# florianwechsung/alfi

Measured on AMD Instinct MI355X. Metric: V-cycles/sec on ldc3d P2-P0 (DoF*smooths/sec in dof_smooths_per_s), higher is better.
Workload: dtype f64

## Files before the change

### alfi_amd/_lib.py

```python
import ctypes
import os

from . import env

_HERE = os.path.dirname(os.path.abspath(__file__))
LIB_PATH = env.hip_lib() or os.path.join(_HERE, "libalfi_hip.so")

c_i32p = ctypes.POINTER(ctypes.c_int32)
c_i64p = ctypes.POINTER(ctypes.c_int64)
c_f64p = ctypes.POINTER(ctypes.c_double)
vp = ctypes.c_void_p


class CsrHost(ctypes.Structure):
    _fields_ = [("nrows", ctypes.c_int64), ("ncols", ctypes.c_int64), ("rowptr", vp), ("colidx", vp), ("vals", vp)]


class BsrHost(ctypes.Structure):
    _fields_ = [("nbrows", ctypes.c_int64), ("nbcols", ctypes.c_int64), ("rowptr", vp), ("colidx", vp), ("vals", vp)]


SIGNATURES = {
    "alfi_ctx_create": (ctypes.c_int, [ctypes.c_int, vp, ctypes.POINTER(vp)]),
    "alfi_ctx_destroy": (ctypes.c_int, [vp]),
# ... 57 lines not shown
    "alfi_level_set_facet_beta": (ctypes.c_int, [vp, vp, ctypes.c_double]),
    "alfi_level_assemble_burman": (ctypes.c_int, [vp, ctypes.c_double, ctypes.c_double, ctypes.c_double, vp, ctypes.c_double,
                                                  ctypes.c_int]),
    "alfi_level_transpose": (ctypes.c_int, [vp]),
    "alfi_level_get_values": (ctypes.c_int, [vp, vp]),
    "alfi_level_size": (ctypes.c_int, [vp, ctypes.POINTER(ctypes.c_int64)]),
    "alfi_spmv": (ctypes.c_int, [vp, vp, vp]),
    "alfi_residual": (ctypes.c_int, [vp, vp, vp, vp]),
    "alfi_patches_set": (ctypes.c_int, [vp, ctypes.c_int64, vp, vp]),
    "alfi_patches_factor": (ctypes.c_int, [vp]),
    "alfi_patches_set_groups": (ctypes.c_int, [vp, vp]),
    "alfi_patches_factor_bytes": (ctypes.c_int, [vp, ctypes.POINTER(ctypes.c_int64)]),
    "alfi_patches_find_groups": (ctypes.c_int, [vp, vp]),
    "alfi_ctx_set_condense_min_bytes": (ctypes.c_int, [vp, ctypes.c_int64]),
    "alfi_patches_condensed": (ctypes.c_int, [vp, ctypes.POINTER(ctypes.c_int)]),
    "alfi_patches_set_storage": (ctypes.c_int, [vp, ctypes.c_int]),
    "alfi_patches_storage": (ctypes.c_int, [vp, ctypes.POINTER(ctypes.c_int)]),
    "alfi_patches_set_macro_storage": (ctypes.c_int, [vp, ctypes.c_int]),
    "alfi_ctx_set_f32_work_bytes": (ctypes.c_int, [vp, ctypes.c_int64]),
    "alfi_ctx_f32_work_bytes": (ctypes.c_int, [vp, ctypes.POINTER(ctypes.c_int64)]),
    "alfi_patches_set_canonical_order": (ctypes.c_int, [vp, vp]),
    "alfi_patch_apply_split": (ctypes.c_int, [vp, ctypes.c_int64, vp, vp]),
    "alfi_patches_check": (ctypes.c_int, [vp, ctypes.POINTER(ctypes.c_double), ctypes.POINTER(ctypes.c_int64),
                                          ctypes.POINTER(ctypes.c_int64), ctypes.POINTER(ctypes.c_double)]),
    "alfi_patches_set_partition_of_unity": (ctypes.c_int, [vp, ctypes.c_int]),
    "alfi_patches_set_multiplicative": (ctypes.c_int, [vp, ctypes.c_int64, vp, ctypes.c_int]),
    "alfi_patches_multiplicative_levels": (ctypes.c_int, [vp, ctypes.POINTER(ctypes.c_int64)]),
    "alfi_patch_apply": (ctypes.c_int, [vp, vp, vp]),
    "alfi_patches_stats": (ctypes.c_int, [vp, ctypes.POINTER(ctypes.c_int64), ctypes.POINTER(ctypes.c_int64),
                                          ctypes.POINTER(ctypes.c_int64)]),
# ... 110 lines not shown
```

### alfi_amd/csrc/api_patches.hip

```cpp
#include <optional>
#include "api_internal.h"
#include "find_groups.h"

static_assert(PLAN_E_ARG == ALFI_E_ARG, "the planners (patch_plan.h) return the C ABI's code");


static void free_f32(alfi_level* L) {
  if (L->inv32 && --L->ctx->f32_levels == 0) {
    dev_free(L->ctx->f32_work);
    L->ctx->f32_work = nullptr;
    L->ctx->f32_work_doubles = 0;
  }
  dev_free(L->inv32);
  dev_free(L->inv32_ptr);
  L->inv32 = nullptr;
  L->inv32_ptr = nullptr;
  L->inv32_floats = 0;
  std::vector<int64_t>().swap(L->f32_ptr);
  if (L->held == HELD_F32) set_held(L, HELD_NONE);
}

static int inv_to_placeholder(alfi_level* L) {
  dev_free(L->inv);
  L->inv = nullptr;
// ... 216 lines not shown
  return 0;
}

int alfi_patches_find_groups(alfi_level* L, int32_t* group_out) {
  alfi_ctx* ctx = L->ctx;
  if (!L->patch_ptr) return alfi_set_error(ctx, ALFI_E_STATE, "alfi_patches_find_groups before alfi_patches_set");
  if (!group_out) return alfi_set_error(ctx, ALFI_E_ARG, "group_out is NULL");
  return find_groups(L, group_out, nullptr);
}

int alfi_ctx_set_condense_min_bytes(alfi_ctx* ctx, int64_t min_bytes) {
  ctx->condense_min_bytes = min_bytes;
  return 0;
}

int alfi_patches_condensed(alfi_level* L, int* mode) {
  if (mode) *mode = !L->cond ? 0 : (cond_by_own_choice(L) ? 2 : 1);
  return 0;
}

int alfi_patches_factor_bytes(alfi_level* L, int64_t* bytes) {
  if (L->held == HELD_F32) {
    *bytes = 4 * L->inv32_floats;
  } else if (wants_f32(L)) {
    std::vector<int64_t> ptr;
    *bytes = 4 * plan_f32_offsets(L->npatch, L->lay.patch_ptr.data(), &ptr);
  } else {
    *bytes = L->cond ? 8 * (L->cplan.mat_doubles + L->cplan.sinv_doubles) : 8 * L->lay.inv_doubles;
  }
  return 0;
// ... 336 lines not shown
```

### alfi_amd/csrc/common.h

```cpp
#pragma once
#include <hip/hip_runtime.h>
#include <atomic>
#include <cstdint>
#include <cstdio>
#include <string>
#include <thread>
#include <vector>
#include "alfi_hip.h"
#include "env.h"
#include "patch_plan.h"

inline std::atomic<int64_t> g_alfi_h2d_bytes{0}, g_alfi_d2h_bytes{0};
inline hipError_t alfi_counted_memcpy(void* dst, const void* src, size_t n, hipMemcpyKind kind) {
  if (kind == hipMemcpyHostToDevice) g_alfi_h2d_bytes += (int64_t)n;
  else if (kind == hipMemcpyDeviceToHost) g_alfi_d2h_bytes += (int64_t)n;
  return hipMemcpy(dst, src, n, kind);
}
inline hipError_t alfi_counted_memcpy_async(void* dst, const void* src, size_t n, hipMemcpyKind kind, hipStream_t s) {
  if (kind == hipMemcpyHostToDevice) g_alfi_h2d_bytes += (int64_t)n;
  else if (kind == hipMemcpyDeviceToHost) g_alfi_d2h_bytes += (int64_t)n;
  return hipMemcpyAsync(dst, src, n, kind, s);
}
#define hipMemcpy(dst, src, n, kind) alfi_counted_memcpy(dst, src, n, kind)
#define hipMemcpyAsync(dst, src, n, kind, stream) alfi_counted_memcpy_async(dst, src, n, kind, stream)
// ... 14 lines not shown
    const int64_t a = t * step, b = a + step < n ? a + step : n;
    if (a < b) th.emplace_back([&fn, a, b] { fn(a, b); });
  }
  fn((int64_t)0, step < n ? step : n);
  for (auto& t : th) t.join();
}

struct alfi_ctx {
  int device = 0;
  hipStream_t stream = nullptr;
  int64_t comm_nhalo = 0, comm_nred = 0, comm_sent = 0;
  int32_t* dev_err = nullptr;
  bool use_graph = false;
  bool block_kernels = true;
  bool block_fused = true;
  int block_lds_bytes = 64 * 1024;
  void* big_arena = nullptr;
  size_t big_arena_bytes = 0;
  void* asm_scratch = nullptr;
  size_t asm_scratch_bytes = 0;
  double* f32_work = nullptr;
  int64_t f32_work_doubles = 0;
  int f32_levels = 0;
  int64_t f32_work_cap = (int64_t)1 << 30;
  int64_t asm_scratch_limit = (int64_t)24 << 30;
  int64_t condense_min_bytes = alfi_default_condense_min_bytes();
  bool own_stream = false;
  std::string err;
  int prof = 0;
  struct EvPair {
// ... 541 lines not shown
```

### alfi_amd/csrc/cond_layout.h

```cpp
#pragma once
#include <cstdint>

#ifdef __HIPCC__
#define ALFI_HD __host__ __device__
#else
#define ALFI_HD
#endif

struct CondChunk {
  int64_t off;
  int64_t ubase;
  int64_t sidx0;
  int64_t stage_off;
  int32_t xq0, xq1;
  int32_t bq0, bq1;
  int32_t e0, ne;
  int32_t u0, nu;
  int32_t nI;
  int32_t xp0, bp0;
  int32_t pad;
};

#ifndef ALFI_COND_SIGMA_ROWS
#define ALFI_COND_SIGMA_ROWS 64
#endif
constexpr int COND_SIGMA_ROWS = ALFI_COND_SIGMA_ROWS;

constexpr int64_t COND_PER_PATCH_MIN = 1024;

ALFI_HD inline int cond_patch_waves(int max_pairs) {
#ifdef ALFI_COND_WAVES_FORCE
  (void)max_pairs;
  return ALFI_COND_WAVES_FORCE;
#else
  return max_pairs <= 64 ? 1 : max_pairs <= 128 ? 2 : max_pairs <= 256 ? 4 : 8;
#endif
}

ALFI_HD inline int cond_ldim(int rows) { return (rows + 1) & ~1; }
ALFI_HD inline int cond_pairs(int rows) { return (rows + 1) / 2; }
ALFI_HD inline int64_t cond_group_doubles(int m, int sc) {
  return (int64_t)cond_ldim(m) * m + (int64_t)cond_ldim(sc) * m + (int64_t)cond_ldim(m) * sc;
}
```

### alfi_amd/csrc/host_assemble.cpp

```cpp
#include <algorithm>
#include <cmath>
#include <cstdint>
#include <cstring>
#include <utility>
#include <vector>
#include <omp.h>

#include "find_groups.h"
#include "patch_plan.h"

extern "C" {

int alfi_host_node_graph(int64_t ncell, int nloc, const int32_t* cell_nodes, int64_t nnode, int32_t* rowptr,
                         int32_t* colidx) {
  std::vector<int64_t> nptr(nnode + 1, 0);
  for (int64_t c = 0; c < ncell; ++c)
    for (int a = 0; a < nloc; ++a) nptr[cell_nodes[c * nloc + a] + 1]++;
  for (int64_t i = 0; i < nnode; ++i) nptr[i + 1] += nptr[i];
  std::vector<int32_t> ncells(nptr[nnode]);
  {
    std::vector<int64_t> fill(nptr.begin(), nptr.end() - 1);
    for (int64_t c = 0; c < ncell; ++c)
      for (int a = 0; a < nloc; ++a) ncells[fill[cell_nodes[c * nloc + a]]++] = (int32_t)c;
  }
// ... 744 lines not shown
  ALFI_PLAN_TABLE(cond, dofs); ALFI_PLAN_TABLE(cond, slot); ALFI_PLAN_TABLE(cond, gptr); ALFI_PLAN_TABLE(cond, g_off);
  ALFI_PLAN_TABLE(cond, g_m); ALFI_PLAN_TABLE(cond, g_sc); ALFI_PLAN_TABLE(cond, g_uoff); ALFI_PLAN_TABLE(cond, g_mat);
  ALFI_PLAN_TABLE(cond, g_sidx); ALFI_PLAN_TABLE(cond, sidx); ALFI_PLAN_TABLE(cond, p_nI); ALFI_PLAN_TABLE(cond, sptr);
  ALFI_PLAN_TABLE(cond, sinv_ptr); ALFI_PLAN_TABLE(cond, s_uptr); ALFI_PLAN_TABLE(cond, s_uidx); ALFI_PLAN_TABLE(cond, order);
  ALFI_PLAN_TABLE(cond, chptr); ALFI_PLAN_TABLE(cond, ch_patch); ALFI_PLAN_TABLE(cond, ch_row); ALFI_PLAN_TABLE(cond, uptr);
  ALFI_PLAN_TABLE(cond, u_dst); ALFI_PLAN_TABLE(cond, xp_ptr); ALFI_PLAN_TABLE(cond, xp_grp); ALFI_PLAN_TABLE(cond, g_xp);
  ALFI_PLAN_TABLE(cond, bp_ptr); ALFI_PLAN_TABLE(cond, bp_grp); ALFI_PLAN_TABLE(cond, g_bp); ALFI_PLAN_TABLE(cond, gcptr);
  ALFI_PLAN_TABLE(cond, gc);
  ALFI_PLAN_SCALAR(cond, ngroups); ALFI_PLAN_SCALAR(cond, mat_doubles); ALFI_PLAN_SCALAR(cond, sinv_doubles);
  ALFI_PLAN_SCALAR(cond, lds_bytes); ALFI_PLAN_SCALAR(cond, lds_front);
  ALFI_PLAN_SCALAR(cond, lds_back); ALFI_PLAN_SCALAR(cond, lds_gfront); ALFI_PLAN_SCALAR(cond, lds_gback);
  ALFI_PLAN_SCALAR(cond, max_s); ALFI_PLAN_SCALAR(cond, max_m); ALFI_PLAN_SCALAR(cond, max_pairs); ALFI_PLAN_SCALAR(cond, umax);
  return h;
}

alfi_host_plan* alfi_host_plan_sweep(int bs, int64_t nbrows, int64_t npatch, const int64_t* patch_ptr, const int32_t* patch_dofs,
                                     const int32_t* rowptr, const int32_t* colidx, int64_t nit, const int64_t* iterset,
                                     int symmetrise) {
  alfi_host_plan* h = new alfi_host_plan();
  bool big = false;
  h->rc = check_sweep(bs, npatch, patch_ptr, patch_dofs, SMALL_PATCH_MAX, nit, iterset, &big, &h->err);
  if (h->rc == 0)
    h->rc = plan_sweep(bs, nbrows, npatch, patch_ptr, patch_dofs, rowptr, colidx, nit, iterset, symmetrise != 0, big, &h->sweep,
                       &h->err);
  if (h->rc != 0) return h;
  ALFI_PLAN_TABLE(sweep, seq); ALFI_PLAN_TABLE(sweep, wave_ptr); ALFI_PLAN_TABLE(sweep, items); ALFI_PLAN_TABLE(sweep, pred0);
  ALFI_PLAN_TABLE(sweep, succ_ptr); ALFI_PLAN_TABLE(sweep, succ); ALFI_PLAN_TABLE(sweep, rowtab);
  ALFI_PLAN_SCALAR(sweep, big); ALFI_PLAN_SCALAR(sweep, nitems);
  return h;
}
// ... 19 lines not shown
```

### alfi_amd/csrc/kernels_bigpatch.hip

```cpp
#include <algorithm>
#include <cstdlib>
#include <vector>
#include "common.h"
#include "row_piece.h"
#include "cond_apply.h"

constexpr int BIG_NB = 64;
constexpr int BIG_MAX_NP = PATCH_MAX;

template <int BS>
__global__ __launch_bounds__(256) void big_gather_kernel(int64_t p0, const int32_t* __restrict__ rowptr,
                                                          const int32_t* __restrict__ colidx,
                                                          const double* __restrict__ vals, int flat,
                                                          const int64_t* __restrict__ patch_ptr,
                                                          const int32_t* __restrict__ patch_dofs,
                                                          const int64_t* __restrict__ scr_ptr, double* __restrict__ scr) {
  __shared__ int32_t dofs_s[BIG_MAX_NP];
  const int64_t p = p0 + blockIdx.y;
  const int64_t off = patch_ptr[p];
  const int n = (int)(patch_ptr[p + 1] - off);
  const int N = (n + BIG_NB - 1) / BIG_NB * BIG_NB;
  double* S = scr + scr_ptr[blockIdx.y];
  for (int i = threadIdx.x; i < n; i += 256) dofs_s[i] = patch_dofs[off + i];
  const int chunk = (N + gridDim.x - 1) / gridDim.x;
// ... 751 lines not shown
    const double* B = cd.mat + cd.g_mat[g] + (int64_t)ldm * m;
    const double* W = B + (int64_t)ldsc * m;
    const int32_t* si = cd.sidx + cd.g_sidx[g];
    for (int e = threadIdx.x; e < sc * sc; e += 256) {
      const int i = e % sc, j = e / sc;
      double acc = 0.0;
      for (int k = 0; k < m; ++k) acc = __builtin_fma(B[(int64_t)k * ldsc + i], W[(int64_t)j * ldm + k], acc);
      S[(int64_t)si[i] * N + si[j]] -= acc;
    }
    __syncthreads();
  }
}



template <bool NT, int COND_WAVES, int RU>
__global__ __launch_bounds__(64 * COND_WAVES) void cond_front_kernel(int64_t p0, int64_t p1, CondDev cd,
                                                                     const int64_t* __restrict__ patch_ptr,
                                                                     const int64_t* __restrict__ stage_ptr,
                                                                     const double* __restrict__ x, double* __restrict__ stage,
                                                                     int ordered) {
  extern __shared__ double cond_dsmem[];
  constexpr int NT_ = 64 * COND_WAVES;
  if (p0 + blockIdx.x >= p1) return;
  const int64_t p = ordered ? cd.order[blockIdx.x] : p0 + blockIdx.x;
  const int64_t off = patch_ptr[p];
  const int n = (int)(patch_ptr[p + 1] - off);
  const int nI = cd.p_nI[p];
  const int s = n - nI;
  const int64_t uo0 = cd.uptr[p];
  double* xs = cond_dsmem;
  double* ts = xs + n;
  double* us = ts + nI;
  for (int i0 = threadIdx.x; i0 < n; i0 += 4 * NT_) {
    int32_t d[4];
#pragma unroll
    for (int u = 0; u < 4; ++u) d[u] = (i0 + u * NT_ < n) ? cd.dofs[off + i0 + u * NT_] : 0;
    double v[4];
#pragma unroll
    for (int u = 0; u < 4; ++u) v[u] = (i0 + u * NT_ < n) ? x[d[u]] : 0.0;
#pragma unroll
    for (int u = 0; u < 4; ++u)
      if (i0 + u * NT_ < n) xs[i0 + u * NT_] = v[u];
  }
  __syncthreads();
  double* tmp = cd.tmp + off;
  const int64_t xp0 = cd.xp_ptr[p], bp0 = cd.bp_ptr[p];
  const int nxp = (int)(cd.xp_ptr[p + 1] - xp0), nbp = (int)(cd.bp_ptr[p + 1] - bp0);
  for (int q0 = 0; q0 < nxp; q0 += NT_) {
    const int q = q0 + threadIdx.x;
    const bool act = q < nxp;
    const int32_t g = act ? cd.xp_grp[xp0 + q] : (int32_t)cd.gptr[p];
    const int m = cd.g_m[g], o = cd.g_off[g], i = 2 * (q - cd.g_xp[g]);
    double t0 = 0.0, t1 = 0.0;
    cond_row2_dot<NT, RU>(cd.mat + cd.g_mat[g] + i, cond_ldim(m), act ? m : 0, xs + o, t0, t1);
    if (act) {
      ts[o + i] = t0;
      tmp[o + i] = t0;
      if (i + 1 < m) {
        ts[o + i + 1] = t1;
        tmp[o + i + 1] = t1;
      }
    }
  }
  __syncthreads();
  for (int q0 = 0; q0 < nbp; q0 += NT_) {
    const int q = q0 + threadIdx.x;
    const bool act = q < nbp;
    const int32_t g = act ? cd.bp_grp[bp0 + q] : (int32_t)cd.gptr[p];
    const int m = cd.g_m[g], sc = cd.g_sc[g], j = 2 * (q - cd.g_bp[g]);
    const int64_t ue = uo0 + cd.g_uoff[g] + j;
    const int32_t d0 = act ? cd.u_dst[ue] : 0, d1 = (act && j + 1 < sc) ? cd.u_dst[ue + 1] : 0;
    double u0 = 0.0, u1 = 0.0;
    cond_row2_dot<NT, RU>(cd.mat + cd.g_mat[g] + (int64_t)cond_ldim(m) * m + j, cond_ldim(sc), act ? m : 0,
                          ts + cd.g_off[g], u0, u1);
    if (act) {
      us[d0] = u0;
      if (j + 1 < sc) us[d1] = u1;
    }
  }
  __syncthreads();
  const int64_t srow0 = cd.sptr[p];
  const int32_t qb = cd.s_uptr[srow0];
  double* rhs = stage + stage_ptr[p] + nI;
  for (int i = threadIdx.x; i < s; i += NT_) {
    double acc = xs[nI + i];
    const int32_t qe = cd.s_uptr[srow0 + i + 1] - qb;
    for (int32_t q = cd.s_uptr[srow0 + i] - qb; q < qe; ++q) acc -= us[q];
    rhs[i] = acc;
  }
}

template <bool NT>
__global__ __launch_bounds__(256) void cond_sigma_kernel(int64_t c0, CondDev cd, const int64_t* __restrict__ patch_ptr,
                                                         const int64_t* __restrict__ stage_ptr,
                                                         const double* __restrict__ stage) {
  extern __shared__ double cond_dsmem[];
  const int64_t c = c0 + blockIdx.x;
  const int64_t p = cd.ch_patch[c];
  const int r0 = cd.ch_row[c];
  const int64_t off = patch_ptr[p];
  const int n = (int)(patch_ptr[p + 1] - off);
  const int nI = cd.p_nI[p];
// ... 27 lines not shown
                                                                    const int64_t* __restrict__ stage_ptr,
                                                                    double* __restrict__ stage, int ordered) {
  extern __shared__ double cond_dsmem[];
  constexpr int NT_ = 64 * COND_WAVES;
  if (p0 + blockIdx.x >= p1) return;
  const int64_t p = ordered ? cd.order[blockIdx.x] : p0 + blockIdx.x;
  const int64_t off = patch_ptr[p];
  const int n = (int)(patch_ptr[p + 1] - off);
  const int nI = cd.p_nI[p];
  const int s = n - nI;
  const int uo = (int)(cd.uptr[p + 1] - cd.uptr[p]);
  const int64_t g0 = cd.gptr[p];
  double* ys = cond_dsmem;
  double* yg = ys + s;
  const double* tmp = cd.tmp + off;
  for (int i = threadIdx.x; i < s; i += NT_) ys[i] = tmp[nI + i];
  const int32_t* si = cd.sidx + (uo > 0 ? cd.g_sidx[g0] : 0);
  int32_t sq[4];
#pragma unroll
  for (int u = 0; u < 4; ++u) sq[u] = (threadIdx.x + u * NT_ < uo) ? si[threadIdx.x + u * NT_] : 0;
  __syncthreads();
#pragma unroll
  for (int u = 0; u < 4; ++u)
    if (threadIdx.x + u * NT_ < uo) yg[threadIdx.x + u * NT_] = ys[sq[u]];
  for (int q = threadIdx.x + 4 * NT_; q < uo; q += NT_) yg[q] = ys[si[q]];
  __syncthreads();
  double* out = stage + stage_ptr[p];
  const int64_t xp0 = cd.xp_ptr[p];
  const int nxp = (int)(cd.xp_ptr[p + 1] - xp0);
  for (int q0 = 0; q0 < nxp; q0 += NT_) {
    const int q = q0 + threadIdx.x;
    const bool act = q < nxp;
    const int32_t g = act ? cd.xp_grp[xp0 + q] : (int32_t)g0;
    const int m = cd.g_m[g], sc = cd.g_sc[g], o = cd.g_off[g], i = 2 * (q - cd.g_xp[g]);
    const int ldm = cond_ldim(m);
    const double tg0 = act ? tmp[o + i] : 0.0, tg1 = (act && i + 1 < m) ? tmp[o + i + 1] : 0.0;
    const int32_t sl0 = act ? cd.slot[off + o + i] : 0, sl1 = (act && i + 1 < m) ? cd.slot[off + o + i + 1] : 0;
    double y0 = 0.0, y1 = 0.0;
    cond_row2_dot<NT, RU>(cd.mat + cd.g_mat[g] + (int64_t)ldm * m + (int64_t)cond_ldim(sc) * m + i, ldm, act ? sc : 0,
                          yg + cd.g_uoff[g], y0, y1);
    if (act) {
      out[sl0] = tg0 - y0;
      if (i + 1 < m) out[sl1] = tg1 - y1;
    }
  }
  for (int i = threadIdx.x; i < s; i += NT_) out[cd.slot[off + nI + i]] = ys[i];
}

template <bool NT>
__device__ __forceinline__ void cond_row2_prefetch(const double* __restrict__ M, int ld, int kn, big_d2 (&a)[COND_U]) {
#pragma unroll
  for (int u = 0; u < COND_U; ++u) {
    const big_d2* q = reinterpret_cast<const big_d2*>(M + (int64_t)u * ld);
    const big_d2 z = {0.0, 0.0};
    a[u] = (u < kn) ? (NT ? __builtin_nontemporal_load(q) : *q) : z;
  }
// ... 441 lines not shown
    const size_t lds_f = (size_t)L->cplan.lds_gfront, lds_b = (size_t)L->cplan.lds_gback;
    const size_t lds_s = (size_t)(L->cplan.max_s + 2 + COND_SIGMA_ROWS) * sizeof(double);
    if (k1 > k0)
      hipLaunchKernelGGL((cond_gfront_kernel<false>), dim3((unsigned)(k1 - k0)), dim3(256), lds_f, ctx->stream, k0, L->cd, x);
    if (c1 > c0)
      hipLaunchKernelGGL((cond_gsigma_kernel<true>), dim3((unsigned)(c1 - c0)), dim3(256), lds_s, ctx->stream, c0, L->cd,
                         L->patch_ptr, L->stage_ptr, x, L->stage);
    if (k1 > k0)
      hipLaunchKernelGGL((cond_gback_kernel<false>), dim3((unsigned)(k1 - k0)), dim3(256), lds_b, ctx->stream, k0, L->cd,
                         L->stage);
    ALFI_HIP_CHECK(ctx, hipGetLastError());
    return 0;
  }
  const size_t lds_f = (size_t)L->cplan.lds_front, lds_s = (size_t)(L->cplan.max_s + 2) * sizeof(double);
  const size_t lds_b = (size_t)L->cplan.lds_back;
#define ALFI_COND_LAUNCH3(WV)                                                                                             \
  do {                                                                                                                    \
    if (lds_f > 64 * 1024)                                                                                                \
      ALFI_HIP_CHECK(ctx, hipFuncSetAttribute(reinterpret_cast<const void*>(&cond_front_kernel<false, WV, 8>),            \
                                              hipFuncAttributeMaxDynamicSharedMemorySize, (int)lds_f));                   \
    hipLaunchKernelGGL((cond_front_kernel<false, WV, 8>), dim3(grid.x), dim3(64 * WV), lds_f, ctx->stream, p0, p1, L->cd, \
                       L->patch_ptr, L->stage_ptr, x, L->stage, ordered);                                                 \
    if (c1 > c0)                                                                                                          \
      hipLaunchKernelGGL((cond_sigma_kernel<true>), dim3((unsigned)(c1 - c0)), dim3(256), lds_s, ctx->stream, c0, L->cd,  \
                         L->patch_ptr, L->stage_ptr, L->stage);                                                           \
    if (lds_b > 64 * 1024)                                                                                                \
      ALFI_HIP_CHECK(ctx, hipFuncSetAttribute(reinterpret_cast<const void*>(&cond_back_kernel<false, WV, 8>),             \
                                              hipFuncAttributeMaxDynamicSharedMemorySize, (int)lds_b));                   \
    hipLaunchKernelGGL((cond_back_kernel<false, WV, 8>), dim3(grid.x), dim3(64 * WV), lds_b, ctx->stream, p0, p1, L->cd,  \
                       L->patch_ptr, L->stage_ptr, L->stage, ordered);                                                    \
  } while (0)
#ifdef ALFI_COND_WAVES_FORCE
  ALFI_COND_LAUNCH3(ALFI_COND_WAVES_FORCE);
#else
  switch (cond_patch_waves(L->cplan.max_pairs)) {
    case 1: ALFI_COND_LAUNCH3(1); break;
    case 2: ALFI_COND_LAUNCH3(2); break;
    case 4: ALFI_COND_LAUNCH3(4); break;
    default: ALFI_COND_LAUNCH3(8); break;
  }
#endif
#undef ALFI_COND_LAUNCH3
  ALFI_HIP_CHECK(ctx, hipGetLastError());
  return 0;
}

#include "mf_coarse.h"
```

### alfi_amd/csrc/patch_plan.h

```cpp
#pragma once
#include <algorithm>
#include <climits>
#include <cstdarg>
#include <cstdint>
#include <cstdio>
#include <string>
#include <vector>
#include "cond_layout.h"

#pragma GCC visibility push(hidden)

constexpr int PLAN_E_ARG = -2;
constexpr int SMALL_PATCH_MAX = 160;
constexpr int PATCH_MAX = 4096;
constexpr int COND_LDS_MAX_BYTES = 150 * 1024;
constexpr int COND_GROUP_MAX = 64;
constexpr int COND_CHUNK_PAIRS = 256;
constexpr int MULT_WAVE_NODES = 64;

inline int plan_fail(std::string* err, const char* fmt, ...) {
  char buf[1024];
  va_list ap;
  va_start(ap, fmt);
  vsnprintf(buf, sizeof(buf), fmt, ap);
// ... 135 lines not shown
  std::vector<int32_t> dofs, slot;
  std::vector<int64_t> gptr, g_mat, g_sidx;
  std::vector<int32_t> g_off, g_m, g_sc, g_uoff, g_xp, g_bp;
  std::vector<int32_t> sidx;
  std::vector<int32_t> p_nI, order;
  std::vector<int64_t> sptr, sinv_ptr, uptr, xp_ptr, bp_ptr;
  std::vector<int32_t> s_uptr, s_uidx, u_dst;
  std::vector<int64_t> chptr, gcptr;
  std::vector<int32_t> ch_patch, ch_row, xp_grp, bp_grp;
  std::vector<CondChunk> gc;
  int64_t ngroups = 0, mat_doubles = 0, sinv_doubles = 0;
  int lds_bytes = 0, lds_front = 0, lds_back = 0, lds_gfront = 0, lds_gback = 0;
  int max_s = 0;
  int max_m = 0;
  int max_pairs = 0;
  int umax = 0;

  void release_tables() {
    CondPlan keep;
    keep.sptr.swap(sptr); keep.gptr.swap(gptr); keep.chptr.swap(chptr); keep.gcptr.swap(gcptr);
    keep.ngroups = ngroups; keep.mat_doubles = mat_doubles; keep.sinv_doubles = sinv_doubles;
    keep.lds_bytes = lds_bytes; keep.lds_front = lds_front; keep.lds_back = lds_back;
    keep.lds_gfront = lds_gfront; keep.lds_gback = lds_gback;
    keep.max_s = max_s; keep.max_m = max_m; keep.max_pairs = max_pairs; keep.umax = umax;
    *this = std::move(keep);
  }
};

inline int plan_condensed(int bs, int64_t nb, int64_t npatch, const int64_t* pp, const int32_t* pd, const int32_t* group,
                          const int32_t* rowptr, const int32_t* colidx, int sigma_rows, CondPlan* out, std::string* err) {
  const int64_t sum_n = pp[npatch];
  std::vector<int32_t> c_dofs(sum_n), c_slot(sum_n), g_off, g_m, g_sc, g_uoff, sidx, p_nI(npatch), s_uptr, s_uidx;
  std::vector<int64_t> gptr(npatch + 1, 0), g_mat, g_sidx, sptr(npatch + 1, 0), sinv_ptr(npatch + 1, 0);
  std::vector<int32_t> node_pos(nb, -1);
  int64_t mat_off = 0, sinv_off = 0;
  int lds_max = 0, umax = 0, smax = 0;
  s_uptr.push_back(0);
  for (int64_t p = 0; p < npatch; ++p) {
    const int64_t off = pp[p];
// ... 92 lines not shown
  if (s_uidx.empty()) s_uidx.push_back(0);
  std::vector<int32_t> order((size_t)npatch);
  {
    std::vector<int64_t> pbytes((size_t)npatch, 0);
    for (int64_t p = 0; p < npatch; ++p) {
      const int64_t s = sptr[p + 1] - sptr[p];
      pbytes[p] = s * s;
      for (int64_t g = gptr[p]; g < gptr[p + 1]; ++g) pbytes[p] += cond_group_doubles(g_m[g], g_sc[g]);
    }
    for (int64_t p = 0; p < npatch; ++p) order[p] = (int32_t)p;
    std::stable_sort(order.begin(), order.end(), [&](int32_t a, int32_t b) { return pbytes[a] > pbytes[b]; });
  }
  std::vector<int32_t> ch_patch, ch_row, xp_grp, bp_grp, g_xp(g_m.size()), g_bp(g_m.size()), u_dst;
  std::vector<int64_t> chptr((size_t)npatch + 1, 0), uptr((size_t)npatch + 1, 0), xp_ptr((size_t)npatch + 1, 0),
      bp_ptr((size_t)npatch + 1, 0);
  int lds_front = 0, lds_back = 0, max_pairs = 0;
  for (int64_t p = 0; p < npatch; ++p) {
    const int s = (int)(sptr[p + 1] - sptr[p]), ld = (s + 1) & ~1;
    for (int r = 0; r < ld; r += sigma_rows) {
      ch_patch.push_back((int32_t)p);
      ch_row.push_back(r);
    }
    chptr[p + 1] = (int64_t)ch_patch.size();
    int uo = 0, xp = 0, bp = 0;
    for (int64_t g = gptr[p]; g < gptr[p + 1]; ++g) {
      g_xp[g] = xp;
      g_bp[g] = bp;
      for (int i = 0; i < cond_pairs(g_m[g]); ++i) xp_grp.push_back((int32_t)g);
      for (int j = 0; j < cond_pairs(g_sc[g]); ++j) bp_grp.push_back((int32_t)g);
      xp += cond_pairs(g_m[g]);
      bp += cond_pairs(g_sc[g]);
      uo += g_sc[g];
    }
    uptr[p + 1] = uptr[p] + uo;
    xp_ptr[p + 1] = xp_ptr[p] + xp;
    bp_ptr[p + 1] = bp_ptr[p] + bp;
    const int32_t qb = s_uptr[sptr[p]], qe = s_uptr[sptr[p + 1]];
    if (qe - qb != uo) return plan_fail(err, "patch %lld: inconsistent skeleton contributions", (long long)p);
    u_dst.resize((size_t)uptr[p + 1]);
    for (int32_t q = qb; q < qe; ++q) u_dst[uptr[p] + s_uidx[q]] = q - qb;
    max_pairs = std::max(max_pairs, std::max(xp, bp));
    lds_front = std::max(lds_front, (int)((pp[p + 1] - pp[p] + p_nI[p] + uo + 2) * (int64_t)sizeof(double)));
    lds_back = std::max(lds_back, (int)((s + uo + 2) * (int64_t)sizeof(double)));
  }
  if (ch_patch.empty()) { ch_patch.push_back(0); ch_row.push_back(0); }
  if (xp_grp.empty()) xp_grp.push_back(0);
  if (bp_grp.empty()) bp_grp.push_back(0);
  if (u_dst.empty()) u_dst.push_back(0);
  if (lds_front > COND_LDS_MAX_BYTES) return plan_fail(err, "condensed apply would need %d bytes of LDS per patch", lds_front);
  std::vector<CondChunk> gc;
  std::vector<int64_t> gcptr((size_t)npatch + 1, 0), stage_off((size_t)npatch + 1, 0);
  for (int64_t p = 0; p < npatch; ++p)
    stage_off[p + 1] = stage_off[p] + ((pp[p + 1] - pp[p] + 1) & ~(int64_t)1);
  int lds_gf = 0, lds_gb = 0;
  for (int64_t p = 0; p < npatch; ++p) {
    int64_t g = gptr[p];
// ... 22 lines not shown
  if (xp_ptr[npatch] > INT32_MAX || bp_ptr[npatch] > INT32_MAX)
    return plan_fail(err, "condensed factors: too many row pairs on one level");
  if (gc.empty()) gc.push_back(CondChunk());
  CondPlan& o = *out;
  o.ngroups = (int64_t)g_off.size();
  o.mat_doubles = mat_off;
  o.sinv_doubles = sinv_off;
  o.lds_bytes = lds_max;
  o.lds_front = lds_front;
  o.lds_back = lds_back;
  o.lds_gfront = lds_gf + 16;
  o.lds_gback = lds_gb + 16;
  o.max_s = smax;
  o.max_m = g_m.empty() ? 0 : *std::max_element(g_m.begin(), g_m.end());
  o.max_pairs = max_pairs;
  o.umax = umax;
  o.dofs = std::move(c_dofs); o.slot = std::move(c_slot);
  o.gptr = std::move(gptr); o.g_mat = std::move(g_mat); o.g_sidx = std::move(g_sidx);
  o.g_off = std::move(g_off); o.g_m = std::move(g_m); o.g_sc = std::move(g_sc); o.g_uoff = std::move(g_uoff);
  o.g_xp = std::move(g_xp); o.g_bp = std::move(g_bp);
  o.sidx = std::move(sidx);
  o.p_nI = std::move(p_nI); o.order = std::move(order);
  o.sptr = std::move(sptr); o.sinv_ptr = std::move(sinv_ptr); o.uptr = std::move(uptr);
  o.xp_ptr = std::move(xp_ptr); o.bp_ptr = std::move(bp_ptr);
  o.s_uptr = std::move(s_uptr); o.s_uidx = std::move(s_uidx); o.u_dst = std::move(u_dst);
  o.chptr = std::move(chptr); o.gcptr = std::move(gcptr);
  o.ch_patch = std::move(ch_patch); o.ch_row = std::move(ch_row); o.xp_grp = std::move(xp_grp); o.bp_grp = std::move(bp_grp);
  o.gc = std::move(gc);
  return 0;
}
// ... 118 lines not shown
```

### alfi_amd/hip.py

```python
import ctypes
import numpy as np

from . import _lib, env
from ._lib import BsrHost, CsrHost, vp


class AlfiHipError(RuntimeError):
    code = None


E_ARG, E_STATE = -2, -3


def _ptr(a):
    return None if a is None else a.ctypes.data_as(vp)


class Context(object):
    def __init__(self, device=0, stream=None):
        self.lib = _lib.load()
        h = vp()
        rc = self.lib.alfi_ctx_create(int(device), vp(stream) if stream else None, ctypes.byref(h))
        if rc != 0:
            raise AlfiHipError("alfi_ctx_create failed (%d): %s -- alfi_amd needs an MI355X; there is no CPU fallback"
# ... 16 lines not shown
            self.h = None

    def set_assembly_scratch(self, max_bytes):
        self.check(self.lib.alfi_ctx_set_assembly_scratch(self.h, int(max_bytes)))

    def set_f32_work_bytes(self, n):
        self.check(self.lib.alfi_ctx_set_f32_work_bytes(self.h, int(n)))

    def f32_work_bytes(self):
        b = ctypes.c_int64()
        self.check(self.lib.alfi_ctx_f32_work_bytes(self.h, ctypes.byref(b)))
        return b.value

    def set_condense_min_bytes(self, min_bytes):
        self.check(self.lib.alfi_ctx_set_condense_min_bytes(self.h, int(min_bytes)))

    def set_comm(self, callback, dred_ptr, dred_len):
        self.check(self.lib.alfi_ctx_set_comm(self.h, ctypes.cast(callback, vp), None, vp(int(dred_ptr)), int(dred_len)))

    def comm_init(self, unique_id, rank, nranks):
        buf = ctypes.create_string_buffer(bytes(unique_id), _lib.COMM_ID_BYTES)
        self.check(self.lib.alfi_ctx_comm_init(self.h, ctypes.cast(buf, vp), int(rank), int(nranks)))

    def comm_allow_self(self, on=True):
        self.check(self.lib.alfi_ctx_comm_allow_self(self.h, 1 if on else 0))

    def comm_size(self):
        r, n = ctypes.c_int(), ctypes.c_int()
        self.check(self.lib.alfi_ctx_comm_size(self.h, ctypes.byref(r), ctypes.byref(n)))
        return r.value, n.value
# ... 970 lines not shown
```

### include/alfi_hip.h

```cpp
#ifndef ALFI_HIP_H
#define ALFI_HIP_H
#include <stdint.h>

#ifdef __cplusplus
extern "C" {
#endif

#define ALFI_OK 0
#define ALFI_E_HIP -1
#define ALFI_E_ARG -2
#define ALFI_E_STATE -3
#define ALFI_E_SINGULAR -4
#define ALFI_E_COMM -5

typedef struct alfi_ctx alfi_ctx;
typedef struct alfi_level alfi_level;
typedef struct alfi_transfer alfi_transfer;
typedef struct alfi_mg alfi_mg;

int alfi_ctx_create(int device, void* stream, alfi_ctx** out);
int alfi_ctx_destroy(alfi_ctx* ctx);
int alfi_ctx_sync(alfi_ctx* ctx);
const char* alfi_last_error(alfi_ctx* ctx);
int alfi_malloc(alfi_ctx* ctx, int64_t bytes, void** dptr);
// ... 78 lines not shown
int alfi_level_set_facet_beta(alfi_level* lvl, const double* beta_host, double scale);
int alfi_level_transpose(alfi_level* lvl);
int alfi_level_get_values(alfi_level* lvl, double* bvals_host);
int alfi_level_size(alfi_level* lvl, int64_t* n);
int alfi_level_id(alfi_level* lvl, int* id);
int alfi_spmv(alfi_level* lvl, const double* dx, double* dy);
int alfi_residual(alfi_level* lvl, const double* db, const double* dx, double* dr);

int alfi_patches_set(alfi_level* lvl, int64_t npatch, const int64_t* patch_ptr_host, const int32_t* patch_dofs_host);
int alfi_patches_factor(alfi_level* lvl);
int alfi_patches_set_groups(alfi_level* lvl, const int32_t* group_host);
int alfi_patches_factor_bytes(alfi_level* lvl, int64_t* bytes);
int alfi_patches_find_groups(alfi_level* lvl, int32_t* group_out_host);
int alfi_ctx_set_condense_min_bytes(alfi_ctx* ctx, int64_t min_bytes);
int alfi_patches_condensed(alfi_level* lvl, int* mode);
#define ALFI_STORAGE_F64 0
#define ALFI_STORAGE_F32 1
int alfi_patches_set_storage(alfi_level* lvl, int dtype);
int alfi_patches_storage(alfi_level* lvl, int* dtype);
int alfi_patches_set_macro_storage(alfi_level* lvl, int dtype);
int alfi_ctx_set_f32_work_bytes(alfi_ctx* ctx, int64_t bytes);
int alfi_ctx_f32_work_bytes(alfi_ctx* ctx, int64_t* bytes);
int alfi_patches_set_canonical_order(alfi_level* lvl, const int32_t* rank_host);
int alfi_patch_apply_split(alfi_level* lvl, int64_t split, const double* x_dev, double* y_dev);
int alfi_patches_check(alfi_level* lvl, double* worst_residual, int64_t* flagged, int64_t* repaired, double* worst_after);
int alfi_patch_apply(alfi_level* lvl, const double* dx, double* dy);
int alfi_patches_set_partition_of_unity(alfi_level* lvl, int on);
int alfi_patches_set_multiplicative(alfi_level* lvl, int64_t nit, const int64_t* iterset_host, int symmetrise);
int alfi_patches_multiplicative_levels(alfi_level* lvl, int64_t* nwave);
int alfi_patches_stats(alfi_level* lvl, int64_t* npatch, int64_t* sum_n, int64_t* sum_n2);
// ... 113 lines not shown
```

Measured before the change: 8.543.

## Split condensed front/back wave counts and prefetch per-thread group metadata

Wave count for the condensed front and back kernels is now chosen separately (with an API override), and the sigma launch is pulled out of the combined macro. Both kernels hoist the per-thread group metadata (matrix offset, dims, scatter targets, slot and tmp values) into registers before the first barrier, overlapping those dependent loads with the LDS fill. Matrix addressing switches to a per-patch base pointer plus 32-bit offsets. The aim is to cut dependent global-load latency and 64-bit address arithmetic in the inner dot products, at the cost of more registers per thread. The default rule gives the same waves for front and back, since both use max(xpairs, bpairs).

After: 8.364. -2.1%, worse.

```diff
diff --git a/alfi_amd/_lib.py b/alfi_amd/_lib.py
--- a/alfi_amd/_lib.py
+++ b/alfi_amd/_lib.py
@@ -95,6 +95,8 @@
     "alfi_patches_find_groups": (ctypes.c_int, [vp, vp]),
     "alfi_ctx_set_condense_min_bytes": (ctypes.c_int, [vp, ctypes.c_int64]),
     "alfi_patches_condensed": (ctypes.c_int, [vp, ctypes.POINTER(ctypes.c_int)]),
+    "alfi_ctx_set_cond_waves": (ctypes.c_int, [vp, ctypes.c_int, ctypes.c_int]),
+    "alfi_ctx_cond_waves": (ctypes.c_int, [vp, ctypes.POINTER(ctypes.c_int), ctypes.POINTER(ctypes.c_int)]),
     "alfi_patches_set_storage": (ctypes.c_int, [vp, ctypes.c_int]),
     "alfi_patches_storage": (ctypes.c_int, [vp, ctypes.POINTER(ctypes.c_int)]),
     "alfi_patches_set_macro_storage": (ctypes.c_int, [vp, ctypes.c_int]),
diff --git a/alfi_amd/csrc/api_patches.hip b/alfi_amd/csrc/api_patches.hip
--- a/alfi_amd/csrc/api_patches.hip
+++ b/alfi_amd/csrc/api_patches.hip
@@ -254,6 +254,22 @@
   return 0;
 }
 
+int alfi_ctx_set_cond_waves(alfi_ctx* ctx, int front, int back) {
+  if (!ctx) return alfi_set_error(nullptr, ALFI_E_ARG, "NULL context");
+  auto ok = [](int w) { return w == 0 || w == 1 || w == 2 || w == 4 || w == 8; };
+  if (!ok(front) || !ok(back))
+    return alfi_set_error(ctx, ALFI_E_ARG, "alfi_ctx_set_cond_waves(%d, %d): 0 (the rule), 1, 2, 4 or 8 waves per patch", front, back);
+  ctx->cond_waves_front = front;
+  ctx->cond_waves_back = back;
+  return 0;
+}
+int alfi_ctx_cond_waves(alfi_ctx* ctx, int* front, int* back) {
+  if (!ctx) return alfi_set_error(nullptr, ALFI_E_ARG, "NULL context");
+  if (front) *front = ctx->cond_waves_front;
+  if (back) *back = ctx->cond_waves_back;
+  return 0;
+}
+
 int alfi_patches_condensed(alfi_level* L, int* mode) {
   if (mode) *mode = !L->cond ? 0 : (cond_by_own_choice(L) ? 2 : 1);
   return 0;
diff --git a/alfi_amd/csrc/common.h b/alfi_amd/csrc/common.h
--- a/alfi_amd/csrc/common.h
+++ b/alfi_amd/csrc/common.h
@@ -52,6 +52,7 @@
   bool use_graph = false;
   bool block_kernels = true;
   bool block_fused = true;
+  int cond_waves_front = 0, cond_waves_back = 0;
   int block_lds_bytes = 64 * 1024;
   void* big_arena = nullptr;
   size_t big_arena_bytes = 0;
diff --git a/alfi_amd/csrc/cond_layout.h b/alfi_amd/csrc/cond_layout.h
--- a/alfi_amd/csrc/cond_layout.h
+++ b/alfi_amd/csrc/cond_layout.h
@@ -37,6 +37,14 @@
 #endif
 }
 
+ALFI_HD inline int cond_pairs_waves(int pairs) { return pairs <= 64 ? 1 : pairs <= 128 ? 2 : pairs <= 256 ? 4 : 8; }
+ALFI_HD inline int cond_front_waves(int max_xpairs, int max_bpairs) {
+  return cond_pairs_waves(max_xpairs > max_bpairs ? max_xpairs : max_bpairs);
+}
+ALFI_HD inline int cond_back_waves(int max_xpairs, int max_bpairs) {
+  return cond_pairs_waves(max_xpairs > max_bpairs ? max_xpairs : max_bpairs);
+}
+
 ALFI_HD inline int cond_ldim(int rows) { return (rows + 1) & ~1; }
 ALFI_HD inline int cond_pairs(int rows) { return (rows + 1) / 2; }
 ALFI_HD inline int64_t cond_group_doubles(int m, int sc) {
diff --git a/alfi_amd/csrc/host_assemble.cpp b/alfi_amd/csrc/host_assemble.cpp
--- a/alfi_amd/csrc/host_assemble.cpp
+++ b/alfi_amd/csrc/host_assemble.cpp
@@ -782,6 +782,10 @@
   return h;
 }
 
+int alfi_host_cond_patch_waves(int max_pairs) { return cond_patch_waves(max_pairs); }
+int alfi_host_cond_front_waves(int max_xpairs, int max_bpairs) { return cond_front_waves(max_xpairs, max_bpairs); }
+int alfi_host_cond_back_waves(int max_xpairs, int max_bpairs) { return cond_back_waves(max_xpairs, max_bpairs); }
+
 alfi_host_plan* alfi_host_plan_sweep(int bs, int64_t nbrows, int64_t npatch, const int64_t* patch_ptr, const int32_t* patch_dofs,
                                      const int32_t* rowptr, const int32_t* colidx, int64_t nit, const int64_t* iterset,
                                      int symmetrise) {
diff --git a/alfi_amd/csrc/kernels_bigpatch.hip b/alfi_amd/csrc/kernels_bigpatch.hip
--- a/alfi_amd/csrc/kernels_bigpatch.hip
+++ b/alfi_amd/csrc/kernels_bigpatch.hip
@@ -789,6 +789,66 @@
 
 
 
+template <bool NT, int RU>
+__device__ __forceinline__ void cond_row2_dot_at(const double* __restrict__ base, uint32_t eo, int ld, int kn,
+                                                 const double* __restrict__ v, double& acc0, double& acc1) {
+  const int kmax = cond_wave_max(kn);
+  for (int k = 0; k < kmax; k += RU) {
+    big_d2 a[RU];
+#pragma unroll
+    for (int u = 0; u < RU; ++u) {
+      const uint32_t byte = (eo + (uint32_t)((k + u) * ld)) * 8u;
+      const big_d2* q = reinterpret_cast<const big_d2*>(reinterpret_cast<const char*>(base) + byte);
+      const big_d2 z = {0.0, 0.0};
+      a[u] = (k + u < kn) ? (NT ? __builtin_nontemporal_load(q) : *q) : z;
+    }
+#pragma unroll
+    for (int u = 0; u < RU; ++u) {
+      const double vk = (k + u < kn) ? v[k + u] : 0.0;
+      acc0 = __builtin_fma(a[u].x, vk, acc0);
+      acc1 = __builtin_fma(a[u].y, vk, acc1);
+    }
+  }
+}
+
+struct CondXRow {
+  int m, sc, o, i, uoff;
+  uint32_t mat;
+};
+struct CondBRow {
+  int m, sc, o, j;
+  uint32_t mat;
+  int32_t d0, d1;
+};
+__device__ __forceinline__ CondXRow cond_xrow(const CondDev& cd, int64_t xp0, int nxp, int64_t mat0, int q) {
+  CondXRow r = {0, 0, 0, 0, 0, 0u};
+  if (q < nxp) {
+    const int32_t g = cd.xp_grp[xp0 + q];
+    r.m = cd.g_m[g];
+    r.sc = cd.g_sc[g];
+    r.o = cd.g_off[g];
+    r.i = 2 * (q - cd.g_xp[g]);
+    r.uoff = cd.g_uoff[g];
+    r.mat = (uint32_t)(cd.g_mat[g] - mat0);
+  }
+  return r;
+}
+__device__ __forceinline__ CondBRow cond_brow(const CondDev& cd, int64_t bp0, int nbp, int64_t mat0, int64_t uo0, int q) {
+  CondBRow r = {0, 0, 0, 0, 0u, 0, 0};
+  if (q < nbp) {
+    const int32_t g = cd.bp_grp[bp0 + q];
+    r.m = cd.g_m[g];
+    r.sc = cd.g_sc[g];
+    r.o = cd.g_off[g];
+    r.j = 2 * (q - cd.g_bp[g]);
+    r.mat = (uint32_t)(cd.g_mat[g] - mat0);
+    const int64_t ue = uo0 + cd.g_uoff[g] + r.j;
+    r.d0 = cd.u_dst[ue];
+    r.d1 = r.j + 1 < r.sc ? cd.u_dst[ue + 1] : 0;
+  }
+  return r;
+}
+
 template <bool NT, int COND_WAVES, int RU>
 __global__ __launch_bounds__(64 * COND_WAVES) void cond_front_kernel(int64_t p0, int64_t p1, CondDev cd,
                                                                      const int64_t* __restrict__ patch_ptr,
@@ -807,6 +867,19 @@
   double* xs = cond_dsmem;
   double* ts = xs + n;
   double* us = ts + nI;
+  const int64_t xp0 = cd.xp_ptr[p], bp0 = cd.bp_ptr[p];
+  const int nxp = (int)(cd.xp_ptr[p + 1] - xp0), nbp = (int)(cd.bp_ptr[p + 1] - bp0);
+  const int64_t mat0 = nxp > 0 ? cd.g_mat[cd.gptr[p]] : 0;
+  const double* matp = cd.mat + mat0;
+  const int64_t srow0 = cd.sptr[p];
+  const int32_t qb = cd.s_uptr[srow0];
+  CondXRow xr = cond_xrow(cd, xp0, nxp, mat0, threadIdx.x);
+  CondBRow br = cond_brow(cd, bp0, nbp, mat0, uo0, threadIdx.x);
+  int32_t r0 = 0, r1 = 0;
+  if ((int)threadIdx.x < s) {
+    r0 = cd.s_uptr[srow0 + threadIdx.x] - qb;
+    r1 = cd.s_uptr[srow0 + threadIdx.x + 1] - qb;
+  }
   for (int i0 = threadIdx.x; i0 < n; i0 += 4 * NT_) {
     int32_t d[4];
 #pragma unroll
@@ -820,16 +893,13 @@
   }
   __syncthreads();
   double* tmp = cd.tmp + off;
-  const int64_t xp0 = cd.xp_ptr[p], bp0 = cd.bp_ptr[p];
-  const int nxp = (int)(cd.xp_ptr[p + 1] - xp0), nbp = (int)(cd.bp_ptr[p + 1] - bp0);
   for (int q0 = 0; q0 < nxp; q0 += NT_) {
     const int q = q0 + threadIdx.x;
-    const bool act = q < nxp;
-    const int32_t g = act ? cd.xp_grp[xp0 + q] : (int32_t)cd.gptr[p];
-    const int m = cd.g_m[g], o = cd.g_off[g], i = 2 * (q - cd.g_xp[g]);
+    if (q0 > 0) xr = cond_xrow(cd, xp0, nxp, mat0, q);
+    const int m = xr.m, o = xr.o, i = xr.i;
     double t0 = 0.0, t1 = 0.0;
-    cond_row2_dot<NT, RU>(cd.mat + cd.g_mat[g] + i, cond_ldim(m), act ? m : 0, xs + o, t0, t1);
-    if (act) {
+    cond_row2_dot_at<NT, RU>(matp, xr.mat + i, cond_ldim(m), m, xs + o, t0, t1);
+    if (q < nxp) {
       ts[o + i] = t0;
       tmp[o + i] = t0;
       if (i + 1 < m) {
@@ -841,27 +911,24 @@
   __syncthreads();
   for (int q0 = 0; q0 < nbp; q0 += NT_) {
     const int q = q0 + threadIdx.x;
-    const bool act = q < nbp;
-    const int32_t g = act ? cd.bp_grp[bp0 + q] : (int32_t)cd.gptr[p];
-    const int m = cd.g_m[g], sc = cd.g_sc[g], j = 2 * (q - cd.g_bp[g]);
-    const int64_t ue = uo0 + cd.g_uoff[g] + j;
-    const int32_t d0 = act ? cd.u_dst[ue] : 0, d1 = (act && j + 1 < sc) ? cd.u_dst[ue + 1] : 0;
+    if (q0 > 0) br = cond_brow(cd, bp0, nbp, mat0, uo0, q);
+    const int m = br.m, sc = br.sc, j = br.j;
     double u0 = 0.0, u1 = 0.0;
-    cond_row2_dot<NT, RU>(cd.mat + cd.g_mat[g] + (int64_t)cond_ldim(m) * m + j, cond_ldim(sc), act ? m : 0,
-                          ts + cd.g_off[g], u0, u1);
-    if (act) {
-      us[d0] = u0;
-      if (j + 1 < sc) us[d1] = u1;
-    }
-  }
-  __syncthreads();
-  const int64_t srow0 = cd.sptr[p];
-  const int32_t qb = cd.s_uptr[srow0];
+    cond_row2_dot_at<NT, RU>(matp, br.mat + (uint32_t)(cond_ldim(m) * m) + j, cond_ldim(sc), m, ts + br.o, u0, u1);
+    if (q < nbp) {
+      us[br.d0] = u0;
+      if (j + 1 < sc) us[br.d1] = u1;
+    }
+  }
+  __syncthreads();
   double* rhs = stage + stage_ptr[p] + nI;
   for (int i = threadIdx.x; i < s; i += NT_) {
+    if (i >= NT_) {
+      r0 = cd.s_uptr[srow0 + i] - qb;
+      r1 = cd.s_uptr[srow0 + i + 1] - qb;
+    }
     double acc = xs[nI + i];
-    const int32_t qe = cd.s_uptr[srow0 + i + 1] - qb;
-    for (int32_t q = cd.s_uptr[srow0 + i] - qb; q < qe; ++q) acc -= us[q];
+    for (int32_t q = r0; q < r1; ++q) acc -= us[q];
     rhs[i] = acc;
   }
 }
@@ -919,6 +986,21 @@
   double* ys = cond_dsmem;
   double* yg = ys + s;
   const double* tmp = cd.tmp + off;
+  const int64_t xp0 = cd.xp_ptr[p];
+  const int nxp = (int)(cd.xp_ptr[p + 1] - xp0);
+  const int64_t mat0 = nxp > 0 ? cd.g_mat[g0] : 0;
+  const double* matp = cd.mat + mat0;
+  CondXRow xr = cond_xrow(cd, xp0, nxp, mat0, threadIdx.x);
+  double tg0 = 0.0, tg1 = 0.0;
+  int32_t sl0 = 0, sl1 = 0;
+  if ((int)threadIdx.x < nxp) {
+    tg0 = tmp[xr.o + xr.i];
+    sl0 = cd.slot[off + xr.o + xr.i];
+    if (xr.i + 1 < xr.m) {
+      tg1 = tmp[xr.o + xr.i + 1];
+      sl1 = cd.slot[off + xr.o + xr.i + 1];
+    }
+  }
   for (int i = threadIdx.x; i < s; i += NT_) ys[i] = tmp[nI + i];
   const int32_t* si = cd.sidx + (uo > 0 ? cd.g_sidx[g0] : 0);
   int32_t sq[4];
@@ -931,20 +1013,27 @@
   for (int q = threadIdx.x + 4 * NT_; q < uo; q += NT_) yg[q] = ys[si[q]];
   __syncthreads();
   double* out = stage + stage_ptr[p];
-  const int64_t xp0 = cd.xp_ptr[p];
-  const int nxp = (int)(cd.xp_ptr[p + 1] - xp0);
   for (int q0 = 0; q0 < nxp; q0 += NT_) {
     const int q = q0 + threadIdx.x;
-    const bool act = q < nxp;
-    const int32_t g = act ? cd.xp_grp[xp0 + q] : (int32_t)g0;
-    const int m = cd.g_m[g], sc = cd.g_sc[g], o = cd.g_off[g], i = 2 * (q - cd.g_xp[g]);
+    if (q0 > 0) {
+      xr = cond_xrow(cd, xp0, nxp, mat0, q);
+      tg0 = tg1 = 0.0;
+      sl0 = sl1 = 0;
+      if (q < nxp) {
+        tg0 = tmp[xr.o + xr.i];
+        sl0 = cd.slot[off + xr.o + xr.i];
+        if (xr.i + 1 < xr.m) {
+          tg1 = tmp[xr.o + xr.i + 1];
+          sl1 = cd.slot[off + xr.o + xr.i + 1];
+        }
+      }
+    }
+    const int m = xr.m, sc = xr.sc, i = xr.i;
     const int ldm = cond_ldim(m);
-    const double tg0 = act ? tmp[o + i] : 0.0, tg1 = (act && i + 1 < m) ? tmp[o + i + 1] : 0.0;
-    const int32_t sl0 = act ? cd.slot[off + o + i] : 0, sl1 = (act && i + 1 < m) ? cd.slot[off + o + i + 1] : 0;
     double y0 = 0.0, y1 = 0.0;
-    cond_row2_dot<NT, RU>(cd.mat + cd.g_mat[g] + (int64_t)ldm * m + (int64_t)cond_ldim(sc) * m + i, ldm, act ? sc : 0,
-                          yg + cd.g_uoff[g], y0, y1);
-    if (act) {
+    cond_row2_dot_at<NT, RU>(matp, xr.mat + (uint32_t)(ldm * m + cond_ldim(sc) * m) + i, ldm, q < nxp ? sc : 0, yg + xr.uoff,
+                             y0, y1);
+    if (q < nxp) {
       out[sl0] = tg0 - y0;
       if (i + 1 < m) out[sl1] = tg1 - y1;
     }
@@ -1416,16 +1505,16 @@
   }
   const size_t lds_f = (size_t)L->cplan.lds_front, lds_s = (size_t)(L->cplan.max_s + 2) * sizeof(double);
   const size_t lds_b = (size_t)L->cplan.lds_back;
-#define ALFI_COND_LAUNCH3(WV)                                                                                             \
+#define ALFI_COND_FRONT(WV)                                                                                               \
   do {                                                                                                                    \
     if (lds_f > 64 * 1024)                                                                                                \
       ALFI_HIP_CHECK(ctx, hipFuncSetAttribute(reinterpret_cast<const void*>(&cond_front_kernel<false, WV, 8>),            \
                                               hipFuncAttributeMaxDynamicSharedMemorySize, (int)lds_f));                   \
     hipLaunchKernelGGL((cond_front_kernel<false, WV, 8>), dim3(grid.x), dim3(64 * WV), lds_f, ctx->stream, p0, p1, L->cd, \
                        L->patch_ptr, L->stage_ptr, x, L->stage, ordered);                                                 \
-    if (c1 > c0)                                                                                                          \
-      hipLaunchKernelGGL((cond_sigma_kernel<true>), dim3((unsigned)(c1 - c0)), dim3(256), lds_s, ctx->stream, c0, L->cd,  \
-                         L->patch_ptr, L->stage_ptr, L->stage);                                                           \
+  } while (0)
+#define ALFI_COND_BACK(WV)                                                                                                \
+  do {                                                                                                                    \
     if (lds_b > 64 * 1024)                                                                                                \
       ALFI_HIP_CHECK(ctx, hipFuncSetAttribute(reinterpret_cast<const void*>(&cond_back_kernel<false, WV, 8>),             \
                                               hipFuncAttributeMaxDynamicSharedMemorySize, (int)lds_b));                   \
@@ -1433,16 +1522,28 @@
                        L->patch_ptr, L->stage_ptr, L->stage, ordered);                                                    \
   } while (0)
 #ifdef ALFI_COND_WAVES_FORCE
-  ALFI_COND_LAUNCH3(ALFI_COND_WAVES_FORCE);
+  const int wf = ALFI_COND_WAVES_FORCE, wb = ALFI_COND_WAVES_FORCE;
 #else
-  switch (cond_patch_waves(L->cplan.max_pairs)) {
-    case 1: ALFI_COND_LAUNCH3(1); break;
-    case 2: ALFI_COND_LAUNCH3(2); break;
-    case 4: ALFI_COND_LAUNCH3(4); break;
-    default: ALFI_COND_LAUNCH3(8); break;
-  }
+  const int wf = ctx->cond_waves_front ? ctx->cond_waves_front : cond_front_waves(L->cplan.max_xpairs, L->cplan.max_bpairs);
+  const int wb = ctx->cond_waves_back ? ctx->cond_waves_back : cond_back_waves(L->cplan.max_xpairs, L->cplan.max_bpairs);
 #endif
-#undef ALFI_COND_LAUNCH3
+  switch (wf) {
+    case 1: ALFI_COND_FRONT(1); break;
+    case 2: ALFI_COND_FRONT(2); break;
+    case 4: ALFI_COND_FRONT(4); break;
+    default: ALFI_COND_FRONT(8); break;
+  }
+  if (c1 > c0)
+    hipLaunchKernelGGL((cond_sigma_kernel<true>), dim3((unsigned)(c1 - c0)), dim3(256), lds_s, ctx->stream, c0, L->cd,
+                       L->patch_ptr, L->stage_ptr, L->stage);
+  switch (wb) {
+    case 1: ALFI_COND_BACK(1); break;
+    case 2: ALFI_COND_BACK(2); break;
+    case 4: ALFI_COND_BACK(4); break;
+    default: ALFI_COND_BACK(8); break;
+  }
+#undef ALFI_COND_FRONT
+#undef ALFI_COND_BACK
   ALFI_HIP_CHECK(ctx, hipGetLastError());
   return 0;
 }
diff --git a/alfi_amd/csrc/patch_plan.h b/alfi_amd/csrc/patch_plan.h
--- a/alfi_amd/csrc/patch_plan.h
+++ b/alfi_amd/csrc/patch_plan.h
@@ -173,6 +173,7 @@
   int max_s = 0;
   int max_m = 0;
   int max_pairs = 0;
+  int max_xpairs = 0, max_bpairs = 0;
   int umax = 0;
 
   void release_tables() {
@@ -182,6 +183,7 @@
     keep.lds_bytes = lds_bytes; keep.lds_front = lds_front; keep.lds_back = lds_back;
     keep.lds_gfront = lds_gfront; keep.lds_gback = lds_gback;
     keep.max_s = max_s; keep.max_m = max_m; keep.max_pairs = max_pairs; keep.umax = umax;
+    keep.max_xpairs = max_xpairs; keep.max_bpairs = max_bpairs;
     *this = std::move(keep);
   }
 };
@@ -304,7 +306,7 @@
   std::vector<int32_t> ch_patch, ch_row, xp_grp, bp_grp, g_xp(g_m.size()), g_bp(g_m.size()), u_dst;
   std::vector<int64_t> chptr((size_t)npatch + 1, 0), uptr((size_t)npatch + 1, 0), xp_ptr((size_t)npatch + 1, 0),
       bp_ptr((size_t)npatch + 1, 0);
-  int lds_front = 0, lds_back = 0, max_pairs = 0;
+  int lds_front = 0, lds_back = 0, max_pairs = 0, max_xpairs = 0, max_bpairs = 0;
   for (int64_t p = 0; p < npatch; ++p) {
     const int s = (int)(sptr[p + 1] - sptr[p]), ld = (s + 1) & ~1;
     for (int r = 0; r < ld; r += sigma_rows) {
@@ -330,6 +332,8 @@
     u_dst.resize((size_t)uptr[p + 1]);
     for (int32_t q = qb; q < qe; ++q) u_dst[uptr[p] + s_uidx[q]] = q - qb;
     max_pairs = std::max(max_pairs, std::max(xp, bp));
+    max_xpairs = std::max(max_xpairs, xp);
+    max_bpairs = std::max(max_bpairs, bp);
     lds_front = std::max(lds_front, (int)((pp[p + 1] - pp[p] + p_nI[p] + uo + 2) * (int64_t)sizeof(double)));
     lds_back = std::max(lds_back, (int)((s + uo + 2) * (int64_t)sizeof(double)));
   }
@@ -382,6 +386,8 @@
   o.max_s = smax;
   o.max_m = g_m.empty() ? 0 : *std::max_element(g_m.begin(), g_m.end());
   o.max_pairs = max_pairs;
+  o.max_xpairs = max_xpairs;
+  o.max_bpairs = max_bpairs;
   o.umax = umax;
   o.dofs = std::move(c_dofs); o.slot = std::move(c_slot);
   o.gptr = std::move(gptr); o.g_mat = std::move(g_mat); o.g_sidx = std::move(g_sidx);
diff --git a/alfi_amd/hip.py b/alfi_amd/hip.py
--- a/alfi_amd/hip.py
+++ b/alfi_amd/hip.py
@@ -54,6 +54,14 @@
 
     def set_condense_min_bytes(self, min_bytes):
         self.check(self.lib.alfi_ctx_set_condense_min_bytes(self.h, int(min_bytes)))
+
+    def set_cond_waves(self, front=0, back=0):
+        self.check(self.lib.alfi_ctx_set_cond_waves(self.h, int(front), int(back)))
+
+    def cond_waves(self):
+        f, b = ctypes.c_int(), ctypes.c_int()
+        self.check(self.lib.alfi_ctx_cond_waves(self.h, ctypes.byref(f), ctypes.byref(b)))
+        return f.value, b.value
 
     def set_comm(self, callback, dred_ptr, dred_len):
         self.check(self.lib.alfi_ctx_set_comm(self.h, ctypes.cast(callback, vp), None, vp(int(dred_ptr)), int(dred_len)))
diff --git a/include/alfi_hip.h b/include/alfi_hip.h
--- a/include/alfi_hip.h
+++ b/include/alfi_hip.h
@@ -116,6 +116,8 @@
 int alfi_patches_find_groups(alfi_level* lvl, int32_t* group_out_host);
 int alfi_ctx_set_condense_min_bytes(alfi_ctx* ctx, int64_t min_bytes);
 int alfi_patches_condensed(alfi_level* lvl, int* mode);
+int alfi_ctx_set_cond_waves(alfi_ctx* ctx, int front, int back);
+int alfi_ctx_cond_waves(alfi_ctx* ctx, int* front, int* back);
 #define ALFI_STORAGE_F64 0
 #define ALFI_STORAGE_F32 1
 int alfi_patches_set_storage(alfi_level* lvl, int dtype);
```
